# NVIDIA/k8s-dra-driver

Measured on AMD Instinct MI355X. Metric: gpu_pods_scheduled_per_sec, higher is better.
Workload: dtype n/a; 1 GPU; model=dra-claim-lifecycle/whole, global_batch=5664, seq_len=0, parallelism=plugin-per-gpu x1, inflight=1, cpus=72-79,200-207, hal=amdsmi, pipeline=CEL-alloc + grpc prepare + cdi + checkpoint, unix-socket v1beta1

## Files before the change

### k8s_dra_driver_amd/build_native.py

```python

from __future__ import annotations

import os
import subprocess
import sys
import sysconfig

PKG_DIR = os.path.dirname(os.path.abspath(__file__))
CPP_DIR = os.path.join(PKG_DIR, "cpp")
ROCM = os.environ.get("ROCM_PATH", "/opt/rocm")
GPU_ARCH = os.environ.get("PYTORCH_ROCM_ARCH", "gfx950")


def _ext_suffix() -> str:
    return sysconfig.get_config_var("EXT_SUFFIX") or ".so"


def _pybind_includes() -> list:
    import pybind11

    return [f"-I{pybind11.get_include()}", f"-I{sysconfig.get_paths()['include']}"]


def _needs_build(src: str, out: str) -> bool:
    return not os.path.exists(out) or os.path.getmtime(src) > os.path.getmtime(out)


def _run(cmd: list) -> None:
    print("+", " ".join(cmd), flush=True)
    subprocess.run(cmd, check=True)


def build_amdhal(force: bool = False) -> str:
    src = os.path.join(CPP_DIR, "amdhal.cpp")
    out = os.path.join(PKG_DIR, f"_amdhal{_ext_suffix()}")
    if force or _needs_build(src, out):
        _run(
            ["g++", "-shared", "-fPIC", "-O2", "-std=c++17"]
            + _pybind_includes()
            + [
                f"-I{ROCM}/include",
                src,
                f"-L{ROCM}/lib",
                "-lamd_smi",
                f"-Wl,-rpath,{ROCM}/lib",
                "-o",
                out,
            ]
        )
    return out


def build_amdhal_asan(force: bool = False) -> str:
    src = os.path.join(CPP_DIR, "amdhal.cpp")
    out = os.path.join(PKG_DIR, f"_amdhal_asan{_ext_suffix()}")
    if force or _needs_build(src, out):
        _run(
            [
                "g++",
                "-shared",
                "-fPIC",
                "-g",
                "-O1",
                "-std=c++17",
                "-fsanitize=address",
                "-fno-omit-frame-pointer",
                "-DPYBIND11_MODULE_NAME=_amdhal_asan",
            ]
            + _pybind_includes()
            + [
                f"-I{ROCM}/include",
                src,
                f"-L{ROCM}/lib",
                "-lamd_smi",
                f"-Wl,-rpath,{ROCM}/lib",
                "-o",
                out,
            ]
        )
    return out


def build_hiphealth(force: bool = False) -> str:
    src = os.path.join(CPP_DIR, "hiphealth.hip")
    out = os.path.join(PKG_DIR, f"_hiphealth{_ext_suffix()}")
    if force or _needs_build(src, out):
        hipcc = os.path.join(ROCM, "bin", "hipcc")
        if not os.path.exists(hipcc):
            hipcc = "hipcc"
        _run(
            [
                hipcc,
                f"--offload-arch={GPU_ARCH}",
                "-shared",
                "-fPIC",
                "-O3",
                "-std=c++17",
            ]
            + _pybind_includes()
            + [src, "-o", out]
        )
    return out


def build(force: bool = False) -> None:
    build_amdhal(force)
    build_hiphealth(force)


if __name__ == "__main__":
    build(force="--force" in sys.argv)
```

### k8s_dra_driver_amd/cdi/spec.py

```python

from __future__ import annotations

import json
import os
from dataclasses import dataclass, field
from typing import List

CDI_VERSION_BASE = "0.5.0"
CDI_VERSION_HOSTPATH = "0.6.0"


@dataclass
class DeviceNode:
    path: str
    host_path: str = ""
    dev_type: str = "c"
    permissions: str = "rw"

    def to_json(self) -> dict:
        out: dict = {"path": self.path, "type": self.dev_type}
        if self.host_path and self.host_path != self.path:
            out["hostPath"] = self.host_path
        if self.permissions:
            out["permissions"] = self.permissions
        return out


@dataclass
class Mount:
    host_path: str
    container_path: str
    options: List[str] = field(default_factory=lambda: ["ro", "nosuid", "nodev", "bind"])

    def to_json(self) -> dict:
        return {
            "hostPath": self.host_path,
            "containerPath": self.container_path,
            "options": list(self.options),
        }


@dataclass
class Hook:
    hook_name: str
    path: str
    args: List[str] = field(default_factory=list)

    def to_json(self) -> dict:
        return {"hookName": self.hook_name, "path": self.path, "args": list(self.args)}


@dataclass
class ContainerEdits:
    env: List[str] = field(default_factory=list)
    device_nodes: List[DeviceNode] = field(default_factory=list)
    mounts: List[Mount] = field(default_factory=list)
    hooks: List[Hook] = field(default_factory=list)

    def merge(self, other: "ContainerEdits") -> "ContainerEdits":
        return ContainerEdits(
            env=self.env + other.env,
            device_nodes=self.device_nodes + other.device_nodes,
            mounts=self.mounts + other.mounts,
            hooks=self.hooks + other.hooks,
        )

    def is_empty(self) -> bool:
        return not (self.env or self.device_nodes or self.mounts or self.hooks)

    def to_json(self) -> dict:
        out: dict = {}
        if self.env:
            out["env"] = list(self.env)
        if self.device_nodes:
            out["deviceNodes"] = [d.to_json() for d in self.device_nodes]
        if self.mounts:
            out["mounts"] = [m.to_json() for m in self.mounts]
        if self.hooks:
            out["hooks"] = [h.to_json() for h in self.hooks]
        return out


@dataclass
class CDIDevice:
    name: str
    edits: ContainerEdits

    def to_json(self) -> dict:
        return {"name": self.name, "containerEdits": self.edits.to_json()}


@dataclass
class CDISpec:
    kind: str
    devices: List[CDIDevice] = field(default_factory=list)
    common_edits: ContainerEdits = field(default_factory=ContainerEdits)

    def minimum_version(self) -> str:
        all_edits = [self.common_edits] + [d.edits for d in self.devices]
        for e in all_edits:
            if e.mounts or e.hooks:
                return CDI_VERSION_HOSTPATH
            if any(d.host_path and d.host_path != d.path for d in e.device_nodes):
                return CDI_VERSION_HOSTPATH
        return CDI_VERSION_BASE

    def to_json(self) -> dict:
        out: dict = {
            "cdiVersion": self.minimum_version(),
            "kind": self.kind,
            "devices": [d.to_json() for d in self.devices],
        }
        if not self.common_edits.is_empty():
            out["containerEdits"] = self.common_edits.to_json()
        return out


def qualified_device_id(kind: str, name: str) -> str:
    return f"{kind}={name}"


def write_spec_file(spec: CDISpec, path: str, *, durable: bool = True) -> None:
    from ..utils.atomicfile import atomic_write_text

    atomic_write_text(
        path,
        json.dumps(spec.to_json(), indent=2, sort_keys=True),
        durable=durable,
    )


def read_spec_file(path: str) -> dict:
    with open(path) as f:
        return json.load(f)
```

### k8s_dra_driver_amd/state/checkpoint.py

```python

from __future__ import annotations

import json
import os
import threading
import zlib
from dataclasses import asdict, dataclass, field
from typing import Dict, List, Optional

from ..utils.atomicfile import atomic_write_json, read_json


class CheckpointCorrupt(RuntimeError):
    pass


@dataclass
class PreparedDevice:

    request_names: List[str]
    pool_name: str
    device_name: str
    cdi_device_ids: List[str]
    parent_gpu_index: int = -1
    kind: str = "gpu"
    device_uuid: str = ""
    admin: bool = False


@dataclass
class PreparedClaim:
    claim_uid: str
    namespace: str = ""
    name: str = ""
    devices: List[PreparedDevice] = field(default_factory=list)
    sharing_strategy: str = ""
    timeslice_gpus: List[int] = field(default_factory=list)
    shared_session_id: str = ""
    repartitioned: Dict[str, List[str]] = field(default_factory=dict)
    claim_env: List[str] = field(default_factory=list)
    claim_mounts: List[dict] = field(default_factory=list)

    def to_v1(self) -> dict:
        return asdict(self)

    @classmethod
    def from_v1(cls, d: dict) -> "PreparedClaim":
        import dataclasses

        dev_fields = {f.name for f in dataclasses.fields(PreparedDevice)}
        devs = [
            PreparedDevice(**{k: v for k, v in pd.items() if k in dev_fields})
            for pd in d.pop("devices", [])
        ]
        known = {f.name for f in dataclasses.fields(cls)}
        return cls(devices=devs, **{k: v for k, v in d.items() if k in known})


def _checksum(payload: dict) -> int:
    data = json.dumps(payload, sort_keys=True, separators=(",", ":")).encode()
    return zlib.crc32(data) & 0xFFFFFFFF


class CheckpointStore:

    def __init__(self, root: str):
        self.root = root
        self.claims_dir = os.path.join(root, "claims")
        os.makedirs(self.claims_dir, exist_ok=True)
        self._lock = threading.Lock()
        self._cache: Dict[str, PreparedClaim] = {}
        self._absent: set = set()

    def _path(self, claim_uid: str) -> str:
        safe = claim_uid.replace("/", "_")
        return os.path.join(self.claims_dir, f"{safe}.json")

    SCHEMA_VERSION = 1

    def write(self, claim: PreparedClaim) -> None:
        v1 = claim.to_v1()
        atomic_write_json(
            self._path(claim.claim_uid),
            {
                "version": self.SCHEMA_VERSION,
                "checksum": _checksum(v1),
                "v1": v1,
            },
        )
        with self._lock:
            self._cache[claim.claim_uid] = claim
            self._absent.discard(claim.claim_uid)

    def read(self, claim_uid: str) -> Optional[PreparedClaim]:
        with self._lock:
            cached = self._cache.get(claim_uid)
            if cached is not None:
                return cached
            if claim_uid in self._absent:
                return None
        claim = self._read_disk(claim_uid)
        with self._lock:
            if claim is None:
                self._absent.add(claim_uid)
                if len(self._absent) > 100_000:
                    self._absent.clear()
            else:
                self._cache[claim_uid] = claim
        return claim

    def _read_disk(self, claim_uid: str) -> Optional[PreparedClaim]:
        path = self._path(claim_uid)
        try:
            obj = read_json(path)
        except FileNotFoundError:
            return None
        except (json.JSONDecodeError, OSError) as e:
            raise CheckpointCorrupt(f"{path}: unreadable: {e}") from e
        version = obj.get("version", 1)
        if version > self.SCHEMA_VERSION:
            raise CheckpointCorrupt(
                f"{path}: checkpoint schema v{version} is newer than this "
                f"plugin understands (v{self.SCHEMA_VERSION}) — refusing to "
                "guess (downgrade rollback safety)"
            )
        v1 = obj.get("v1")
        if v1 is None or obj.get("checksum") != _checksum(v1):
            raise CheckpointCorrupt(f"{path}: checksum mismatch")
        return PreparedClaim.from_v1(v1)

    def delete(self, claim_uid: str) -> None:
        with self._lock:
            self._cache.pop(claim_uid, None)
            self._absent.add(claim_uid)
        try:
            os.unlink(self._path(claim_uid))
        except FileNotFoundError:
            pass

    def list_all(self) -> Dict[str, PreparedClaim]:
        out: Dict[str, PreparedClaim] = {}
        for name in sorted(os.listdir(self.claims_dir)):
            if not name.endswith(".json") or name.startswith(".tmp-"):
                continue
            uid = name[: -len(".json")]
            claim = self.read(uid)
            if claim is not None:
                out[claim.claim_uid] = claim
        return out

    def invalidate_cache(self) -> None:
        with self._lock:
            self._cache.clear()
            self._absent.clear()
```

### k8s_dra_driver_amd/utils/atomicfile.py

```python

from __future__ import annotations

import itertools
import json
import os
import threading
from typing import Any

_counter = itertools.count()
_known_dirs = set()
_dirs_lock = threading.Lock()


def _ensure_dir(d: str) -> None:
    if d in _known_dirs:
        return
    os.makedirs(d, exist_ok=True)
    with _dirs_lock:
        _known_dirs.add(d)


def _tmp_name(path: str) -> str:
    d = os.path.dirname(path)
    return os.path.join(d, f".tmp-{os.getpid()}-{next(_counter)}")


def atomic_write_text(path: str, data: str, *, durable: bool = True) -> None:
    d = os.path.dirname(path)
    _ensure_dir(d)
    tmp = _tmp_name(path)
    try:
        fd = os.open(tmp, os.O_WRONLY | os.O_CREAT | os.O_EXCL, 0o644)
    except FileNotFoundError:
        with _dirs_lock:
            _known_dirs.discard(d)
        _ensure_dir(d)
        fd = os.open(tmp, os.O_WRONLY | os.O_CREAT | os.O_EXCL, 0o644)
    try:
        os.write(fd, data.encode())
        if durable:
            os.fsync(fd)
        os.close(fd)
        fd = -1
        os.replace(tmp, path)
    except BaseException:
        if fd >= 0:
            os.close(fd)
        try:
            os.unlink(tmp)
        except OSError:
            pass
        raise


def atomic_write_json(path: str, obj: Any) -> None:
    atomic_write_text(
        path, json.dumps(obj, sort_keys=True, separators=(",", ":"))
    )


def read_json(path: str) -> Any:
    with open(path) as f:
        return json.load(f)
```

### setup.py

```python

import sys

from setuptools import Command, find_packages, setup


class BuildNative(Command):
    description = "build in-tree native extensions (_amdhal, _hiphealth)"
    user_options = [("inplace", "i", "build into the package dir (always on)")]

    def initialize_options(self):
        self.inplace = True

    def finalize_options(self):
        pass

    def run(self):
        sys.path.insert(0, ".")
        from k8s_dra_driver_amd import build_native

        build_native.build()


setup(
    name="k8s-dra-driver-amd",
    version="0.1.0",
    description="MI355X-native Kubernetes Dynamic Resource Allocation driver",
    packages=find_packages(include=["k8s_dra_driver_amd*"]),
    package_data={"k8s_dra_driver_amd": ["*.so"]},
    python_requires=">=3.9",
    cmdclass={"build_ext": BuildNative},
    entry_points={
        "console_scripts": [
            "amd-dra-kubeletplugin=k8s_dra_driver_amd.plugin.main:main",
            "amd-dra-controller=k8s_dra_driver_amd.controller.main:main",
            "amd-dra-ctl=k8s_dra_driver_amd.ctl:main",
            "amd-dra-workload=k8s_dra_driver_amd.workload:main",
            "amd-dra-demo=k8s_dra_driver_amd.demo_runner:main",
        ]
    },
)
```

Baseline: 1925 pods/s.

## Add native C++ claim persistence for JSON encoding, checksum and atomic writes

Adds a pybind11 extension that serialises checkpoint dataclasses and CDI specs straight to JSON bytes, computes the CRC32 checksum in C++, and performs the tmp-write/fsync/rename with the GIL released. Checkpoint reads also go through a native file read. The aim is to cut Python-level json.dumps, asdict conversion and syscall overhead in the prepare path. In exchange it adds a compiled dependency with a Python fallback, and the output must stay byte-compatible with the Python encoder's checksum and format.

```diff
diff --git a/k8s_dra_driver_amd/build_native.py b/k8s_dra_driver_amd/build_native.py
--- a/k8s_dra_driver_amd/build_native.py
+++ b/k8s_dra_driver_amd/build_native.py
@@ -103,9 +103,60 @@
     return out
 
 
+def build_claimio(force: bool = False) -> str:
+    src = os.path.join(CPP_DIR, "claimio.cpp")
+    hdr = os.path.join(CPP_DIR, "claimio_core.hpp")
+    out = os.path.join(PKG_DIR, f"_claimio{_ext_suffix()}")
+    if force or _needs_build(src, out) or _needs_build(hdr, out):
+        _run(
+            ["g++", "-shared", "-fPIC", "-O2", "-std=c++17"]
+            + _pybind_includes()
+            + [src, "-o", out]
+        )
+    return out
+
+
+def _gcc_file(name: str) -> str:
+    try:
+        out = subprocess.run(
+            ["gcc", f"-print-file-name={name}"],
+            capture_output=True,
+            text=True,
+            check=True,
+        ).stdout.strip()
+    except (OSError, subprocess.CalledProcessError):
+        return ""
+    return out if os.path.isabs(out) else ""
+
+
+def sanitizer_link_flags():
+    if _gcc_file("libasan.a") and _gcc_file("libubsan.a"):
+        return ["-static-libasan", "-static-libubsan"]
+    if _gcc_file("libasan.so") and _gcc_file("libubsan.so"):
+        return []
+    return None
+
+
+def build_claimio_selftest(out: str, sanitize: bool = True) -> str:
+    src = os.path.join(CPP_DIR, "claimio_selftest.cpp")
+    flags = ["-g", "-O1", "-std=c++17"]
+    if sanitize:
+        link = sanitizer_link_flags()
+        if link is None:
+            raise RuntimeError("gcc has no ASan/UBSan runtime installed")
+        flags += [
+            "-fsanitize=address,undefined",
+            "-fno-sanitize-recover=undefined",
+            "-fno-omit-frame-pointer",
+        ] + link
+    _run(["g++"] + flags + [src, "-o", out])
+    return out
+
+
 def build(force: bool = False) -> None:
     build_amdhal(force)
     build_hiphealth(force)
+    build_claimio(force)
 
 
 if __name__ == "__main__":
diff --git a/k8s_dra_driver_amd/cdi/spec.py b/k8s_dra_driver_amd/cdi/spec.py
--- a/k8s_dra_driver_amd/cdi/spec.py
+++ b/k8s_dra_driver_amd/cdi/spec.py
@@ -121,13 +121,9 @@
 
 
 def write_spec_file(spec: CDISpec, path: str, *, durable: bool = True) -> None:
-    from ..utils.atomicfile import atomic_write_text
+    from ..utils.atomicfile import atomic_write_bytes, encode_json
 
-    atomic_write_text(
-        path,
-        json.dumps(spec.to_json(), indent=2, sort_keys=True),
-        durable=durable,
-    )
+    atomic_write_bytes(path, encode_json(spec.to_json(), 2), durable=durable)
 
 
 def read_spec_file(path: str) -> dict:
diff --git a/k8s_dra_driver_amd/cpp/claimio.cpp b/k8s_dra_driver_amd/cpp/claimio.cpp
--- /dev/null
+++ b/k8s_dra_driver_amd/cpp/claimio.cpp
@@ -0,0 +1,298 @@
+
+#include <pybind11/pybind11.h>
+
+#include <algorithm>
+#include <string>
+#include <unordered_map>
+#include <utility>
+#include <vector>
+
+#include "claimio_core.hpp"
+
+namespace py = pybind11;
+
+namespace {
+
+constexpr int kMaxDepth = 200;
+
+struct DcField {
+    PyObject* name;
+    std::string key;
+};
+
+std::unordered_map<PyTypeObject*, std::vector<DcField>> g_dataclasses;
+
+bool type_error(const char* what, PyObject* o) {
+    PyErr_Format(PyExc_TypeError, "_claimio: %s (%.200s)", what,
+                 Py_TYPE(o)->tp_name);
+    return false;
+}
+
+bool append_str(std::string& out, PyObject* s) {
+#if PY_VERSION_HEX < 0x030C0000
+    if (PyUnicode_READY(s) < 0) return false;
+#endif
+    const void* data = PyUnicode_DATA(s);
+    size_t n = static_cast<size_t>(PyUnicode_GET_LENGTH(s));
+    switch (PyUnicode_KIND(s)) {
+        case PyUnicode_1BYTE_KIND:
+            claimio::append_escaped(out, static_cast<const uint8_t*>(data), n);
+            return true;
+        case PyUnicode_2BYTE_KIND:
+            claimio::append_escaped(out, static_cast<const uint16_t*>(data), n);
+            return true;
+        case PyUnicode_4BYTE_KIND:
+            claimio::append_escaped(out, static_cast<const uint32_t*>(data), n);
+            return true;
+        default:
+            return type_error("unsupported str storage", s);
+    }
+}
+
+const std::vector<DcField>* dataclass_fields(PyTypeObject* tp, bool* failed) {
+    *failed = false;
+    auto it = g_dataclasses.find(tp);
+    if (it != g_dataclasses.end()) return &it->second;
+    PyObject* tpo = reinterpret_cast<PyObject*>(tp);
+    int has = PyObject_HasAttrString(tpo, "__dataclass_fields__");
+    if (has <= 0) return nullptr;
+    try {
+        py::object fields =
+            py::module_::import("dataclasses").attr("fields")(py::handle(tpo));
+        std::vector<py::object> names;
+        for (py::handle f : fields) {
+            py::object name = f.attr("name");
+            if (!PyUnicode_Check(name.ptr())) return nullptr;
+            names.push_back(std::move(name));
+        }
+        std::sort(names.begin(), names.end(),
+                  [](const py::object& a, const py::object& b) {
+                      return PyUnicode_Compare(a.ptr(), b.ptr()) < 0;
+                  });
+        std::vector<DcField> out;
+        for (auto& n : names) {
+            DcField f;
+            if (!append_str(f.key, n.ptr())) throw py::error_already_set();
+            f.name = n.release().ptr();
+            out.push_back(std::move(f));
+        }
+        Py_INCREF(tpo);
+        return &g_dataclasses.emplace(tp, std::move(out)).first->second;
+    } catch (py::error_already_set& e) {
+        e.restore();
+        *failed = true;
+        return nullptr;
+    }
+}
+
+bool encode_value(PyObject* o, claimio::Emitter& e, int depth);
+
+bool encode_sequence(PyObject* o, claimio::Emitter& e, int depth) {
+    const bool is_list = PyList_Check(o);
+    const size_t n = static_cast<size_t>(is_list ? PyList_GET_SIZE(o)
+                                                 : PyTuple_GET_SIZE(o));
+    e.open('[', n);
+    for (size_t i = 0; i < n; ++i) {
+        if (is_list && i >= static_cast<size_t>(PyList_GET_SIZE(o))) {
+            PyErr_SetString(PyExc_RuntimeError,
+                            "_claimio: list changed size during encoding");
+            return false;
+        }
+        PyObject* item = is_list ? PyList_GET_ITEM(o, i) : PyTuple_GET_ITEM(o, i);
+        Py_INCREF(item);
+        e.item(i);
+        bool ok = encode_value(item, e, depth + 1);
+        Py_DECREF(item);
+        if (!ok) return false;
+    }
+    e.close(']', n);
+    return true;
+}
+
+bool encode_dict(PyObject* o, claimio::Emitter& e, int depth) {
+    std::vector<std::pair<PyObject*, PyObject*>> items;
+    items.reserve(static_cast<size_t>(PyDict_Size(o)));
+    PyObject *k, *v;
+    Py_ssize_t pos = 0;
+    while (PyDict_Next(o, &pos, &k, &v)) {
+        if (!PyUnicode_Check(k)) return type_error("dict key is not a str", k);
+        items.emplace_back(k, v);
+    }
+    for (auto& kv : items) {
+        Py_INCREF(kv.first);
+        Py_INCREF(kv.second);
+    }
+    std::sort(items.begin(), items.end(),
+              [](const std::pair<PyObject*, PyObject*>& a,
+                 const std::pair<PyObject*, PyObject*>& b) {
+                  return PyUnicode_Compare(a.first, b.first) < 0;
+              });
+    bool ok = true;
+    e.open('{', items.size());
+    for (size_t i = 0; ok && i < items.size(); ++i) {
+        e.item(i);
+        ok = append_str(e.out(), items[i].first);
+        if (ok) {
+            e.colon();
+            ok = encode_value(items[i].second, e, depth + 1);
+        }
+    }
+    if (ok) e.close('}', items.size());
+    for (auto& kv : items) {
+        Py_DECREF(kv.first);
+        Py_DECREF(kv.second);
+    }
+    return ok;
+}
+
+bool encode_dataclass(PyObject* o, const std::vector<DcField>& fields,
+                      claimio::Emitter& e, int depth) {
+    e.open('{', fields.size());
+    for (size_t i = 0; i < fields.size(); ++i) {
+        PyObject* v = PyObject_GetAttr(o, fields[i].name);
+        if (!v) return false;
+        e.item(i);
+        e.out().append(fields[i].key);
+        e.colon();
+        bool ok = encode_value(v, e, depth + 1);
+        Py_DECREF(v);
+        if (!ok) return false;
+    }
+    e.close('}', fields.size());
+    return true;
+}
+
+bool encode_value(PyObject* o, claimio::Emitter& e, int depth) {
+    std::string& out = e.out();
+    if (o == Py_None) {
+        out.append("null", 4);
+        return true;
+    }
+    if (o == Py_True) {
+        out.append("true", 4);
+        return true;
+    }
+    if (o == Py_False) {
+        out.append("false", 5);
+        return true;
+    }
+    if (PyUnicode_Check(o)) return append_str(out, o);
+    if (PyLong_Check(o)) {
+        int overflow = 0;
+        long long v = PyLong_AsLongLongAndOverflow(o, &overflow);
+        if (!overflow) {
+            if (v == -1 && PyErr_Occurred()) return false;
+            claimio::append_int(out, v);
+            return true;
+        }
+        PyObject* s = PyLong_Type.tp_repr(o);
+        if (!s) return false;
+        Py_ssize_t len = 0;
+        const char* utf8 = PyUnicode_AsUTF8AndSize(s, &len);
+        if (utf8) out.append(utf8, static_cast<size_t>(len));
+        Py_DECREF(s);
+        return utf8 != nullptr;
+    }
+    if (depth > kMaxDepth) return type_error("nesting too deep", o);
+    if (PyList_Check(o) || PyTuple_Check(o)) return encode_sequence(o, e, depth);
+    if (PyDict_Check(o)) return encode_dict(o, e, depth);
+    if (PyFloat_Check(o)) return type_error("float is left to json.dumps", o);
+    if (!PyType_Check(o)) {
+        bool failed = false;
+        const std::vector<DcField>* fields = dataclass_fields(Py_TYPE(o), &failed);
+        if (failed) return false;
+        if (fields) return encode_dataclass(o, *fields, e, depth);
+    }
+    return type_error("unsupported type", o);
+}
+
+int parse_indent(const py::object& indent) {
+    if (indent.is_none()) return -1;
+    if (!PyLong_Check(indent.ptr()))
+        throw py::type_error("_claimio: indent must be an int or None");
+    long v = PyLong_AsLong(indent.ptr());
+    if (v == -1 && PyErr_Occurred()) throw py::error_already_set();
+    return v < 0 ? 0 : static_cast<int>(std::min<long>(v, 1 << 16));
+}
+
+py::bytes encode(const py::object& obj, const py::object& indent) {
+    claimio::Emitter e(parse_indent(indent));
+    e.out().reserve(1024);
+    if (!encode_value(obj.ptr(), e, 0)) throw py::error_already_set();
+    return py::bytes(e.out());
+}
+
+py::bytes encode_checkpoint(const py::object& claim, long long version) {
+    claimio::Emitter e(-1);
+    std::string& out = e.out();
+    out.reserve(1024);
+    static const char kHead[] = "{\"checksum\":";
+    static const char kMid[] = ",\"v1\":";
+    const size_t slot = sizeof(kHead) - 1 + 10 + sizeof(kMid) - 1;
+    out.assign(slot, ' ');
+    if (!encode_value(claim.ptr(), e, 0)) throw py::error_already_set();
+    const uint32_t crc = claimio::crc32(out.data() + slot, out.size() - slot);
+    std::string head(kHead);
+    claimio::append_uint(head, crc);
+    head.append(kMid);
+    const size_t start = slot - head.size();
+    out.replace(start, head.size(), head);
+    out.append(",\"version\":");
+    claimio::append_int(out, version);
+    out.push_back('}');
+    return py::bytes(out.data() + start, out.size() - start);
+}
+
+py::object fs_path(const py::object& p) {
+    PyObject* b = nullptr;
+    if (!PyUnicode_FSConverter(p.ptr(), &b)) throw py::error_already_set();
+    return py::reinterpret_steal<py::object>(b);
+}
+
+[[noreturn]] void raise_oserror(int err, const py::object& filename) {
+    errno = err;
+    PyErr_SetFromErrnoWithFilenameObject(PyExc_OSError, filename.ptr());
+    throw py::error_already_set();
+}
+
+void write_replace(const py::object& tmp, const py::object& path,
+                   const py::bytes& data, bool durable) {
+    py::object tmp_b = fs_path(tmp), path_b = fs_path(path);
+    const char* tmp_c = PyBytes_AS_STRING(tmp_b.ptr());
+    const char* path_c = PyBytes_AS_STRING(path_b.ptr());
+    const char* buf = PyBytes_AS_STRING(data.ptr());
+    const size_t n = static_cast<size_t>(PyBytes_GET_SIZE(data.ptr()));
+    const char* failed = nullptr;
+    int err;
+    {
+        py::gil_scoped_release nogil;
+        err = claimio::write_replace(tmp_c, path_c, buf, n, durable, &failed);
+    }
+    if (err) raise_oserror(err, failed == path_c ? path : tmp);
+}
+
+py::object read_or_none(const py::object& path) {
+    py::object path_b = fs_path(path);
+    const char* path_c = PyBytes_AS_STRING(path_b.ptr());
+    std::string out;
+    int err;
+    {
+        py::gil_scoped_release nogil;
+        err = claimio::read_file(path_c, out);
+    }
+    if (err == ENOENT) return py::none();
+    if (err) raise_oserror(err, path);
+    return py::bytes(out);
+}
+
+}
+
+PYBIND11_MODULE(_claimio, m) {
+    m.doc() = "native claim persistence: JSON encode, checksum, atomic write";
+    m.def("encode", &encode, py::arg("obj"), py::arg("indent") = py::none());
+    m.def("encode_checkpoint", &encode_checkpoint, py::arg("claim"),
+          py::arg("version"));
+    m.def("write_replace", &write_replace, py::arg("tmp"), py::arg("path"),
+          py::arg("data"), py::arg("durable"));
+    m.def("read_or_none", &read_or_none, py::arg("path"));
+}
diff --git a/k8s_dra_driver_amd/cpp/claimio_core.hpp b/k8s_dra_driver_amd/cpp/claimio_core.hpp
--- /dev/null
+++ b/k8s_dra_driver_amd/cpp/claimio_core.hpp
@@ -0,0 +1,234 @@
+#pragma once
+
+#include <cerrno>
+#include <cstddef>
+#include <cstdint>
+#include <cstring>
+#include <string>
+
+#include <fcntl.h>
+#include <stdio.h>
+#include <sys/types.h>
+#include <unistd.h>
+
+namespace claimio {
+
+
+inline void append_u16_escape(std::string& out, uint32_t v) {
+    static const char hex[] = "0123456789abcdef";
+    char buf[6] = {'\\', 'u', hex[(v >> 12) & 0xf], hex[(v >> 8) & 0xf],
+                   hex[(v >> 4) & 0xf], hex[v & 0xf]};
+    out.append(buf, 6);
+}
+
+inline void append_escaped_cp(std::string& out, uint32_t c) {
+    if (c >= 0x20 && c <= 0x7e && c != '"' && c != '\\') {
+        out.push_back(static_cast<char>(c));
+        return;
+    }
+    switch (c) {
+        case '"': out.append("\\\"", 2); return;
+        case '\\': out.append("\\\\", 2); return;
+        case '\n': out.append("\\n", 2); return;
+        case '\r': out.append("\\r", 2); return;
+        case '\t': out.append("\\t", 2); return;
+        case '\b': out.append("\\b", 2); return;
+        case '\f': out.append("\\f", 2); return;
+        default: break;
+    }
+    if (c >= 0x10000) {
+        uint32_t v = c - 0x10000;
+        append_u16_escape(out, 0xd800 | ((v >> 10) & 0x3ff));
+        append_u16_escape(out, 0xdc00 | (v & 0x3ff));
+    } else {
+        append_u16_escape(out, c);
+    }
+}
+
+template <typename CharT>
+inline void append_escaped(std::string& out, const CharT* s, size_t n) {
+    out.push_back('"');
+    size_t i = 0;
+    while (i < n) {
+        size_t j = i;
+        if (sizeof(CharT) == 1) {
+            while (j < n) {
+                uint32_t c = s[j];
+                if (c < 0x20 || c > 0x7e || c == '"' || c == '\\') break;
+                ++j;
+            }
+            if (j > i) {
+                out.append(reinterpret_cast<const char*>(s) + i, j - i);
+                i = j;
+                continue;
+            }
+        }
+        append_escaped_cp(out, static_cast<uint32_t>(s[i]));
+        ++i;
+    }
+    out.push_back('"');
+}
+
+
+inline void append_int(std::string& out, long long v) {
+    char buf[24];
+    char* p = buf + sizeof(buf);
+    unsigned long long u = v < 0 ? 0ULL - static_cast<unsigned long long>(v)
+                                 : static_cast<unsigned long long>(v);
+    do {
+        *--p = static_cast<char>('0' + u % 10);
+        u /= 10;
+    } while (u);
+    if (v < 0) *--p = '-';
+    out.append(p, static_cast<size_t>(buf + sizeof(buf) - p));
+}
+
+inline void append_uint(std::string& out, unsigned long long u) {
+    char buf[24];
+    char* p = buf + sizeof(buf);
+    do {
+        *--p = static_cast<char>('0' + u % 10);
+        u /= 10;
+    } while (u);
+    out.append(p, static_cast<size_t>(buf + sizeof(buf) - p));
+}
+
+
+class Emitter {
+  public:
+    explicit Emitter(int indent) : indent_(indent), depth_(0) {}
+
+    std::string& out() { return out_; }
+    bool compact() const { return indent_ < 0; }
+
+    void open(char bracket, size_t n) {
+        out_.push_back(bracket);
+        if (n) ++depth_;
+    }
+    void item(size_t i) {
+        if (i) out_.push_back(',');
+        if (indent_ >= 0) newline();
+    }
+    void colon() {
+        if (indent_ >= 0)
+            out_.append(": ", 2);
+        else
+            out_.push_back(':');
+    }
+    void close(char bracket, size_t n) {
+        if (n) {
+            --depth_;
+            if (indent_ >= 0) newline();
+        }
+        out_.push_back(bracket);
+    }
+
+  private:
+    void newline() {
+        out_.push_back('\n');
+        out_.append(static_cast<size_t>(indent_) * depth_, ' ');
+    }
+    std::string out_;
+    int indent_;
+    size_t depth_;
+};
+
+
+struct Crc32Table {
+    uint32_t t[4][256];
+    Crc32Table() {
+        for (uint32_t i = 0; i < 256; ++i) {
+            uint32_t c = i;
+            for (int k = 0; k < 8; ++k) c = (c & 1) ? 0xedb88320u ^ (c >> 1) : c >> 1;
+            t[0][i] = c;
+        }
+        for (uint32_t i = 0; i < 256; ++i)
+            for (int s = 1; s < 4; ++s)
+                t[s][i] = (t[s - 1][i] >> 8) ^ t[0][t[s - 1][i] & 0xff];
+    }
+};
+
+inline uint32_t crc32(const void* data, size_t n) {
+    static const Crc32Table tab;
+    const unsigned char* p = static_cast<const unsigned char*>(data);
+    uint32_t c = 0xffffffffu;
+    while (n >= 4) {
+        c ^= static_cast<uint32_t>(p[0]) | static_cast<uint32_t>(p[1]) << 8 |
+             static_cast<uint32_t>(p[2]) << 16 | static_cast<uint32_t>(p[3]) << 24;
+        c = tab.t[3][c & 0xff] ^ tab.t[2][(c >> 8) & 0xff] ^
+            tab.t[1][(c >> 16) & 0xff] ^ tab.t[0][c >> 24];
+        p += 4;
+        n -= 4;
+    }
+    while (n--) c = tab.t[0][(c ^ *p++) & 0xff] ^ (c >> 8);
+    return c ^ 0xffffffffu;
+}
+
+
+typedef ssize_t (*write_fn_t)(int, const void*, size_t);
+
+inline int write_all(int fd, const char* data, size_t n,
+                     write_fn_t write_fn = ::write) {
+    while (n) {
+        ssize_t w = write_fn(fd, data, n);
+        if (w < 0) {
+            if (errno == EINTR) continue;
+            return errno;
+        }
+        if (w == 0) return EIO;
+        data += w;
+        n -= static_cast<size_t>(w);
+    }
+    return 0;
+}
+
+inline int write_replace(const char* tmp, const char* path, const char* data,
+                         size_t n, bool durable, const char** failed,
+                         write_fn_t write_fn = ::write) {
+    *failed = tmp;
+    int fd;
+    do {
+        fd = ::open(tmp, O_WRONLY | O_CREAT | O_EXCL | O_CLOEXEC, 0644);
+    } while (fd < 0 && errno == EINTR);
+    if (fd < 0) return errno;
+    int err = write_all(fd, data, n, write_fn);
+    if (!err && durable) {
+        int r;
+        do {
+            r = ::fsync(fd);
+        } while (r < 0 && errno == EINTR);
+        if (r < 0) err = errno;
+    }
+    if (::close(fd) < 0 && !err && errno != EINTR) err = errno;
+    if (!err && ::rename(tmp, path) < 0) {
+        err = errno;
+        *failed = path;
+    }
+    if (err) ::unlink(tmp);
+    return err;
+}
+
+inline int read_file(const char* path, std::string& out) {
+    int fd;
+    do {
+        fd = ::open(path, O_RDONLY | O_CLOEXEC);
+    } while (fd < 0 && errno == EINTR);
+    if (fd < 0) return errno;
+    out.clear();
+    char buf[8192];
+    int err = 0;
+    for (;;) {
+        ssize_t r = ::read(fd, buf, sizeof(buf));
+        if (r < 0) {
+            if (errno == EINTR) continue;
+            err = errno;
+            break;
+        }
+        if (r == 0) break;
+        out.append(buf, static_cast<size_t>(r));
+    }
+    ::close(fd);
+    return err;
+}
+
+}
diff --git a/k8s_dra_driver_amd/cpp/claimio_selftest.cpp b/k8s_dra_driver_amd/cpp/claimio_selftest.cpp
--- /dev/null
+++ b/k8s_dra_driver_amd/cpp/claimio_selftest.cpp
@@ -0,0 +1,333 @@
+
+#include "claimio_core.hpp"
+
+#include <cstdio>
+#include <cstdlib>
+#include <string>
+#include <vector>
+
+#include <dirent.h>
+#include <sys/stat.h>
+
+static int g_failures = 0;
+
+#define CHECK(cond)                                                          \
+    do {                                                                     \
+        if (!(cond)) {                                                       \
+            std::fprintf(stderr, "FAIL %s:%d: %s\n", __FILE__, __LINE__,     \
+                         #cond);                                             \
+            ++g_failures;                                                    \
+        }                                                                    \
+    } while (0)
+
+
+static std::string ref_escape_cp(uint32_t c) {
+    char buf[16];
+    switch (c) {
+        case '"': return "\\\"";
+        case '\\': return "\\\\";
+        case '\n': return "\\n";
+        case '\r': return "\\r";
+        case '\t': return "\\t";
+        case '\b': return "\\b";
+        case '\f': return "\\f";
+        default: break;
+    }
+    if (c < 0x20) {
+        std::snprintf(buf, sizeof(buf), "\\u%04x", c);
+        return buf;
+    }
+    if (c <= 0x7e) return std::string(1, static_cast<char>(c));
+    if (c < 0x10000) {
+        std::snprintf(buf, sizeof(buf), "\\u%04x", c);
+        return buf;
+    }
+    uint32_t v = c - 0x10000;
+    std::snprintf(buf, sizeof(buf), "\\u%04x\\u%04x", 0xd800 + (v >> 10),
+                  0xdc00 + (v & 0x3ff));
+    return buf;
+}
+
+template <typename CharT>
+static void check_range(uint32_t lo, uint32_t hi) {
+    for (uint32_t c = lo; c <= hi; ++c) {
+        CharT s[1] = {static_cast<CharT>(c)};
+        std::string got;
+        claimio::append_escaped(got, s, 1);
+        std::string want = "\"" + ref_escape_cp(c) + "\"";
+        if (got != want) {
+            std::fprintf(stderr, "FAIL escape U+%04X width %zu: %s != %s\n", c,
+                         sizeof(CharT), got.c_str(), want.c_str());
+            ++g_failures;
+            return;
+        }
+    }
+    std::vector<CharT> all;
+    std::string want = "\"";
+    for (uint32_t c = lo; c <= hi; ++c) {
+        all.push_back(static_cast<CharT>('a'));
+        all.push_back(static_cast<CharT>(c));
+        want += "a" + ref_escape_cp(c);
+    }
+    want += "\"";
+    std::string got;
+    claimio::append_escaped(got, all.data(), all.size());
+    CHECK(got == want);
+}
+
+static void test_escaper() {
+    check_range<uint8_t>(0x00, 0xff);
+    check_range<uint16_t>(0x0000, 0xffff);
+    check_range<uint32_t>(0x000000, 0x10ffff);
+
+    std::string out;
+    claimio::append_escaped(out, static_cast<const uint8_t*>(nullptr), 0);
+    CHECK(out == "\"\"");
+
+    const uint32_t edges[] = {0x00,   0x1f,   0x20,   0x22,    0x5c,    0x7e,
+                              0x7f,   0x80,   0xff,   0x100,   0x2028,  0xd7ff,
+                              0xd800, 0xdbff, 0xdc00, 0xdfff,  0xe000,  0xffff,
+                              0x10000, 0x1f600, 0x10ffff};
+    out.clear();
+    claimio::append_escaped(out, edges, sizeof(edges) / sizeof(edges[0]));
+    CHECK(out ==
+          "\"\\u0000\\u001f \\\"\\\\~\\u007f\\u0080\\u00ff\\u0100\\u2028\\ud7ff"
+          "\\ud800\\udbff\\udc00\\udfff\\ue000\\uffff\\ud800\\udc00"
+          "\\ud83d\\ude00\\udbff\\udfff\"");
+}
+
+
+static void test_numbers() {
+    struct {
+        long long v;
+        const char* s;
+    } cases[] = {{0, "0"},
+                 {-1, "-1"},
+                 {7, "7"},
+                 {-10, "-10"},
+                 {1234567890123LL, "1234567890123"},
+                 {9223372036854775807LL, "9223372036854775807"},
+                 {-9223372036854775807LL - 1, "-9223372036854775808"}};
+    for (auto& c : cases) {
+        std::string out;
+        claimio::append_int(out, c.v);
+        CHECK(out == c.s);
+    }
+    std::string out;
+    claimio::append_uint(out, 18446744073709551615ULL);
+    CHECK(out == "18446744073709551615");
+
+    CHECK(claimio::crc32("", 0) == 0u);
+    CHECK(claimio::crc32("123456789", 9) == 0xcbf43926u);
+    std::string buf(64, '\0');
+    for (size_t i = 0; i < buf.size(); ++i) buf[i] = static_cast<char>(i * 37 + 1);
+    for (size_t off = 0; off < 4; ++off)
+        for (size_t n = 0; n + off <= buf.size(); ++n) {
+            uint32_t bytewise = 0xffffffffu;
+            for (size_t i = 0; i < n; ++i) {
+                bytewise ^= static_cast<unsigned char>(buf[off + i]);
+                for (int k = 0; k < 8; ++k)
+                    bytewise = (bytewise & 1) ? 0xedb88320u ^ (bytewise >> 1)
+                                              : bytewise >> 1;
+            }
+            CHECK(claimio::crc32(buf.data() + off, n) == (bytewise ^ 0xffffffffu));
+        }
+}
+
+
+static void key(claimio::Emitter& e, size_t i, const char* k) {
+    e.item(i);
+    claimio::append_escaped(e.out(), reinterpret_cast<const uint8_t*>(k),
+                            std::strlen(k));
+    e.colon();
+}
+
+static std::string emit_sample(int indent) {
+    claimio::Emitter e(indent);
+    e.open('{', 4);
+    key(e, 0, "a");
+    e.open('[', 0);
+    e.close(']', 0);
+    key(e, 1, "b");
+    e.open('{', 0);
+    e.close('}', 0);
+    key(e, 2, "c");
+    e.open('[', 3);
+    e.item(0);
+    claimio::append_int(e.out(), 1);
+    e.item(1);
+    e.open('[', 2);
+    e.item(0);
+    claimio::append_int(e.out(), 2);
+    e.item(1);
+    e.open('[', 0);
+    e.close(']', 0);
+    e.close(']', 2);
+    e.item(2);
+    e.open('{', 1);
+    key(e, 0, "d");
+    e.open('{', 0);
+    e.close('}', 0);
+    e.close('}', 1);
+    e.close(']', 3);
+    key(e, 3, "e");
+    e.open('{', 1);
+    key(e, 0, "f");
+    e.open('[', 1);
+    e.item(0);
+    e.open('{', 0);
+    e.close('}', 0);
+    e.close(']', 1);
+    e.close('}', 1);
+    e.close('}', 4);
+    return e.out();
+}
+
+static void test_emitters() {
+    CHECK(emit_sample(-1) ==
+          "{\"a\":[],\"b\":{},\"c\":[1,[2,[]],{\"d\":{}}],\"e\":{\"f\":[{}]}}");
+    CHECK(emit_sample(2) ==
+          "{\n"
+          "  \"a\": [],\n"
+          "  \"b\": {},\n"
+          "  \"c\": [\n"
+          "    1,\n"
+          "    [\n"
+          "      2,\n"
+          "      []\n"
+          "    ],\n"
+          "    {\n"
+          "      \"d\": {}\n"
+          "    }\n"
+          "  ],\n"
+          "  \"e\": {\n"
+          "    \"f\": [\n"
+          "      {}\n"
+          "    ]\n"
+          "  }\n"
+          "}");
+    CHECK(emit_sample(0) ==
+          "{\n\"a\": [],\n\"b\": {},\n\"c\": [\n1,\n[\n2,\n[]\n],\n{\n\"d\": "
+          "{}\n}\n],\n\"e\": {\n\"f\": [\n{}\n]\n}\n}");
+    claimio::Emitter empty_list(2), empty_dict(-1);
+    empty_list.open('[', 0);
+    empty_list.close(']', 0);
+    empty_dict.open('{', 0);
+    empty_dict.close('}', 0);
+    CHECK(empty_list.out() == "[]");
+    CHECK(empty_dict.out() == "{}");
+}
+
+
+static int count_entries(const std::string& dir, const char* prefix) {
+    DIR* d = ::opendir(dir.c_str());
+    if (!d) return -1;
+    int n = 0;
+    while (dirent* ent = ::readdir(d))
+        if (std::strncmp(ent->d_name, prefix, std::strlen(prefix)) == 0) ++n;
+    ::closedir(d);
+    return n;
+}
+
+static int g_write_calls = 0;
+
+static ssize_t stingy_write(int fd, const void* p, size_t n) {
+    if (++g_write_calls % 3 == 0) {
+        errno = EINTR;
+        return -1;
+    }
+    return ::write(fd, p, n < 7 ? n : 7);
+}
+
+static ssize_t failing_write(int fd, const void* p, size_t n) {
+    if (++g_write_calls > 2) {
+        errno = ENOSPC;
+        return -1;
+    }
+    return ::write(fd, p, n < 5 ? n : 5);
+}
+
+static void test_files() {
+    const char* base = std::getenv("TMPDIR");
+    std::string tmpl = std::string(base && *base ? base : "/tmp") + "/claimio-selftest-XXXXXX";
+    std::vector<char> tbuf(tmpl.begin(), tmpl.end());
+    tbuf.push_back('\0');
+    CHECK(::mkdtemp(tbuf.data()) != nullptr);
+    const std::string dir = tbuf.data();
+    const std::string tmp = dir + "/.tmp-1-0", path = dir + "/out.json";
+    const char* failed = nullptr;
+    std::string back;
+
+    for (int durable = 0; durable < 2; ++durable) {
+        std::string data = durable ? "{\"durable\":true}" : "{}";
+        CHECK(claimio::write_replace(tmp.c_str(), path.c_str(), data.data(),
+                                     data.size(), durable != 0, &failed) == 0);
+        CHECK(claimio::read_file(path.c_str(), back) == 0);
+        CHECK(back == data);
+        CHECK(count_entries(dir, ".tmp-") == 0);
+    }
+
+    std::string big(100000, 'x');
+    for (size_t i = 0; i < big.size(); ++i) big[i] = static_cast<char>('a' + i % 26);
+    CHECK(claimio::write_replace(tmp.c_str(), path.c_str(), big.data(),
+                                 big.size(), false, &failed) == 0);
+    CHECK(claimio::read_file(path.c_str(), back) == 0);
+    CHECK(back == big);
+    CHECK(claimio::write_replace(tmp.c_str(), path.c_str(), "", 0, false,
+                                 &failed) == 0);
+    CHECK(claimio::read_file(path.c_str(), back) == 0);
+    CHECK(back.empty());
+
+    g_write_calls = 0;
+    CHECK(claimio::write_replace(tmp.c_str(), path.c_str(), big.data(), 1000,
+                                 false, &failed, stingy_write) == 0);
+    CHECK(g_write_calls > 1000 / 7);
+    CHECK(claimio::read_file(path.c_str(), back) == 0);
+    CHECK(back == big.substr(0, 1000));
+
+    g_write_calls = 0;
+    CHECK(claimio::write_replace(tmp.c_str(), path.c_str(), big.data(), 100,
+                                 false, &failed, failing_write) == ENOSPC);
+    CHECK(failed == tmp.c_str());
+    CHECK(count_entries(dir, ".tmp-") == 0);
+    CHECK(claimio::read_file(path.c_str(), back) == 0);
+    CHECK(back == big.substr(0, 1000));
+
+    const std::string sub = dir + "/busy";
+    CHECK(::mkdir(sub.c_str(), 0755) == 0);
+    CHECK(claimio::write_replace(tmp.c_str(), (sub + "/f").c_str(), "x", 1,
+                                 false, &failed) == 0);
+    const std::string tmp2 = dir + "/.tmp-1-1";
+    int err = claimio::write_replace(tmp2.c_str(), sub.c_str(), "y", 1, false,
+                                     &failed);
+    CHECK(err == EISDIR || err == ENOTEMPTY || err == EEXIST);
+    CHECK(failed == sub.c_str());
+    CHECK(count_entries(dir, ".tmp-") == 0);
+
+    CHECK(claimio::write_replace(path.c_str(), (dir + "/other").c_str(), "z",
+                                 1, false, &failed) == EEXIST);
+    CHECK(claimio::read_file(path.c_str(), back) == 0);
+    const std::string gone = dir + "/gone/.tmp-1-2";
+    CHECK(claimio::write_replace(gone.c_str(), (dir + "/gone/f").c_str(), "z",
+                                 1, true, &failed) == ENOENT);
+    CHECK(failed == gone.c_str());
+    CHECK(claimio::read_file((dir + "/gone/f").c_str(), back) == ENOENT);
+
+    ::unlink((sub + "/f").c_str());
+    ::rmdir(sub.c_str());
+    ::unlink(path.c_str());
+    CHECK(::rmdir(dir.c_str()) == 0);
+}
+
+int main() {
+    test_escaper();
+    test_numbers();
+    test_emitters();
+    test_files();
+    if (g_failures) {
+        std::fprintf(stderr, "claimio_selftest: %d check(s) failed\n", g_failures);
+        return 1;
+    }
+    std::puts("claimio_selftest: OK");
+    return 0;
+}
diff --git a/k8s_dra_driver_amd/state/checkpoint.py b/k8s_dra_driver_amd/state/checkpoint.py
--- a/k8s_dra_driver_amd/state/checkpoint.py
+++ b/k8s_dra_driver_amd/state/checkpoint.py
@@ -8,6 +8,7 @@
 from dataclasses import asdict, dataclass, field
 from typing import Dict, List, Optional
 
+from ..utils import atomicfile
 from ..utils.atomicfile import atomic_write_json, read_json
 
 
@@ -79,15 +80,26 @@
     SCHEMA_VERSION = 1
 
     def write(self, claim: PreparedClaim) -> None:
-        v1 = claim.to_v1()
-        atomic_write_json(
-            self._path(claim.claim_uid),
-            {
-                "version": self.SCHEMA_VERSION,
-                "checksum": _checksum(v1),
-                "v1": v1,
-            },
-        )
+        path = self._path(claim.claim_uid)
+        data = None
+        nat = atomicfile.native()
+        if nat is not None:
+            try:
+                data = nat.encode_checkpoint(claim, self.SCHEMA_VERSION)
+            except TypeError:
+                data = None
+        if data is not None:
+            atomicfile.atomic_write_bytes(path, data)
+        else:
+            v1 = claim.to_v1()
+            atomic_write_json(
+                path,
+                {
+                    "version": self.SCHEMA_VERSION,
+                    "checksum": _checksum(v1),
+                    "v1": v1,
+                },
+            )
         with self._lock:
             self._cache[claim.claim_uid] = claim
             self._absent.discard(claim.claim_uid)
@@ -112,7 +124,14 @@
     def _read_disk(self, claim_uid: str) -> Optional[PreparedClaim]:
         path = self._path(claim_uid)
         try:
-            obj = read_json(path)
+            nat = atomicfile.native()
+            if nat is not None:
+                raw = nat.read_or_none(path)
+                if raw is None:
+                    return None
+                obj = json.loads(raw)
+            else:
+                obj = read_json(path)
         except FileNotFoundError:
             return None
         except (json.JSONDecodeError, OSError) as e:
diff --git a/k8s_dra_driver_amd/utils/atomicfile.py b/k8s_dra_driver_amd/utils/atomicfile.py
--- a/k8s_dra_driver_amd/utils/atomicfile.py
+++ b/k8s_dra_driver_amd/utils/atomicfile.py
@@ -3,13 +3,51 @@
 
 import itertools
 import json
+import logging
 import os
 import threading
 from typing import Any
 
+log = logging.getLogger(__name__)
+
+try:
+    from .. import _claimio as _native_mod
+except ImportError as _e:
+    _native_mod = None
+    _native_import_error = str(_e)
+else:
+    _native_import_error = ""
+
+_native_on = _native_mod is not None
+_fallback_warned = False
+
 _counter = itertools.count()
 _known_dirs = set()
 _dirs_lock = threading.Lock()
+
+
+def set_native(on: bool) -> bool:
+    global _native_on
+    if on and _native_mod is None:
+        raise RuntimeError(
+            f"_claimio extension not available: {_native_import_error}"
+        )
+    prev, _native_on = _native_on, bool(on)
+    return prev
+
+
+def native():
+    global _fallback_warned
+    if _native_on:
+        return _native_mod
+    if not _fallback_warned:
+        _fallback_warned = True
+        log.warning(
+            "claim persistence is running on the pure-Python path (%s); "
+            "expect a slower prepare",
+            _native_import_error or "native path switched off",
+        )
+    return None
 
 
 def _ensure_dir(d: str) -> None:
@@ -25,10 +63,22 @@
     return os.path.join(d, f".tmp-{os.getpid()}-{next(_counter)}")
 
 
-def atomic_write_text(path: str, data: str, *, durable: bool = True) -> None:
+def atomic_write_bytes(path: str, data: bytes, *, durable: bool = True) -> None:
     d = os.path.dirname(path)
     _ensure_dir(d)
     tmp = _tmp_name(path)
+    nat = native()
+    if nat is not None:
+        try:
+            nat.write_replace(tmp, path, data, durable)
+        except FileNotFoundError as e:
+            if e.filename != tmp:
+                raise
+            with _dirs_lock:
+                _known_dirs.discard(d)
+            _ensure_dir(d)
+            nat.write_replace(tmp, path, data, durable)
+        return
     try:
         fd = os.open(tmp, os.O_WRONLY | os.O_CREAT | os.O_EXCL, 0o644)
     except FileNotFoundError:
@@ -37,7 +87,7 @@
         _ensure_dir(d)
         fd = os.open(tmp, os.O_WRONLY | os.O_CREAT | os.O_EXCL, 0o644)
     try:
-        os.write(fd, data.encode())
+        os.write(fd, data)
         if durable:
             os.fsync(fd)
         os.close(fd)
@@ -53,10 +103,24 @@
         raise
 
 
+def atomic_write_text(path: str, data: str, *, durable: bool = True) -> None:
+    atomic_write_bytes(path, data.encode(), durable=durable)
+
+
+def encode_json(obj: Any, indent=None) -> bytes:
+    nat = native()
+    if nat is not None:
+        try:
+            return nat.encode(obj, indent)
+        except TypeError:
+            pass
+    if indent is None:
+        return json.dumps(obj, sort_keys=True, separators=(",", ":")).encode()
+    return json.dumps(obj, indent=indent, sort_keys=True).encode()
+
+
 def atomic_write_json(path: str, obj: Any) -> None:
-    atomic_write_text(
-        path, json.dumps(obj, sort_keys=True, separators=(",", ":"))
-    )
+    atomic_write_bytes(path, encode_json(obj))
 
 
 def read_json(path: str) -> Any:
diff --git a/setup.py b/setup.py
--- a/setup.py
+++ b/setup.py
@@ -5,7 +5,7 @@
 
 
 class BuildNative(Command):
-    description = "build in-tree native extensions (_amdhal, _hiphealth)"
+    description = "build in-tree native extensions (_amdhal, _hiphealth, _claimio)"
     user_options = [("inplace", "i", "build into the package dir (always on)")]
 
     def initialize_options(self):
```

Measured after the change: 2144 pods/s, median of 6. +11.4%, better.
